# CODEJIN/multi_speaker_tts

Hardware: AMD Instinct MI355X
Metric: mel-frames/sec (train step) at batch 32x(128 tok,800 mel) (higher is better)
Workload: dtype f32

## Files before the change

multi_speaker_tts_amd/csrc/gemm_split.inc:

```

typedef __bf16 gs_bf16x8 __attribute__((ext_vector_type(8)));
typedef __bf16 gs_bf16x4 __attribute__((ext_vector_type(4)));
constexpr int GS_BM = 128, GS_LD = 40;
constexpr int GS_PLANE = 128 * GS_LD;

struct Split3 { gs_bf16x4 hi, mid, lo; };
__device__ __forceinline__ uint32_t gs_cvt_pk(float a, float b) {
    uint32_t r;
    asm("v_cvt_pk_bf16_f32 %0, %1, %2" : "=v"(r) : "v"(a), "v"(b));
    return r;
}
__device__ __forceinline__ float gs_sub(float a, uint32_t b_bits) {
    float r;
    asm("v_sub_f32 %0, %1, %2" : "=v"(r) : "v"(a), "v"(b_bits));
    return r;
}
__device__ __forceinline__ void gs_split2(float x0, float x1, uint32_t& hi, uint32_t& mid, uint32_t& lo) {
    hi = gs_cvt_pk(x0, x1);
    x0 = gs_sub(x0, hi << 16); x1 = gs_sub(x1, hi & 0xffff0000u);
    mid = gs_cvt_pk(x0, x1);
    x0 = gs_sub(x0, mid << 16); x1 = gs_sub(x1, mid & 0xffff0000u);
    lo = gs_cvt_pk(x0, x1);
}
__device__ __forceinline__ Split3 gs_split4(float a, float b, float c, float d) {
    uint2 h, m, l;
    gs_split2(a, b, h.x, m.x, l.x);
    gs_split2(c, d, h.y, m.y, l.y);
    Split3 s;
    s.hi = __builtin_bit_cast(gs_bf16x4, h); s.mid = __builtin_bit_cast(gs_bf16x4, m); s.lo = __builtin_bit_cast(gs_bf16x4, l);
    return s;
}
template <int PLANE>
struct SplitPlanes {
    static __device__ __forceinline__ void put(__bf16* __restrict__ p, float a, float b, float c, float d) {
        const Split3 s = gs_split4(a, b, c, d);
        *reinterpret_cast<gs_bf16x4*>(p) = s.hi;
        *reinterpret_cast<gs_bf16x4*>(p + PLANE) = s.mid;
        *reinterpret_cast<gs_bf16x4*>(p + 2 * PLANE) = s.lo;
    }
};

template <bool VEC, bool WIN> using GsLoaderKC = TileLoaderKC<8, 4, 32, GS_LD, SplitPlanes<GS_PLANE>, VEC, WIN>;
template <bool VEC, bool WIN> using GsLoaderMC = TileLoaderMC<8, GS_LD, SplitPlanes<GS_PLANE>, VEC, WIN>;

#ifdef GS_STAMP
#define GS_BAR(slot) do { if (stamp) { const unsigned long long t0_ = __builtin_readcyclecounter(); gemm_barrier(); acc_wait += __builtin_readcyclecounter() - t0_; } else gemm_barrier(); } while (0)
#else
#define GS_BAR(slot) gemm_barrier()
#endif

__device__ __forceinline__ int tiles_m_of(const GemmArgs& g) { return (g.M + GS_BM - 1) / GS_BM; }
constexpr int GS_NPROD = 6;
constexpr int GS_BUF = 6 * GS_PLANE;
constexpr size_t GS_LDS_BYTES = 2 * GS_BUF * sizeof(__bf16);

constexpr int GS_THREADS = 768;
template <class LoadFn, class StoreFn>
__device__ __forceinline__ void gs_produce(LoadFn load, StoreFn store, __bf16* lds0, int kbeg, int nt2) {
    float4 r[2][4];
    load(r[0], kbeg);
    load(r[1], kbeg + BK);
    store(r[0], lds0);
    load(r[0], kbeg + 2 * BK);
    gemm_barrier();
    for (int t = 0; t < nt2; t += 2) {
        store(r[1], lds0 + GS_BUF);
        load(r[1], kbeg + (t + 3) * BK);
        gemm_barrier();
        store(r[0], lds0);
        load(r[0], kbeg + (t + 4) * BK);
        gemm_barrier();
    }
}

template <bool TA, bool TB, bool VEC, bool WIN>
__global__ __launch_bounds__(GS_THREADS) void gemm_split_kernel(GemmArgs g) {
    extern __shared__ __attribute__((aligned(16))) __bf16 gs_lds[];

    const int tiles_n = (g.N + BN - 1) / BN;
    int tile = blockIdx.x, piece = -1;
    if (tile < g.body) {
        tile = gemm_xcd_tile(tile, g.body);
    } else {
        const int u = tile - g.body;
        tile = g.body + u / g.tail_s;
        piece = u % g.tail_s;
    }
    int tile_m = tile / tiles_n, tile_n = tile % tiles_n;
    if (g.band > 0) {
        const int per_band = g.band * tiles_m_of(g), b = tile / per_band, r = tile - b * per_band;
        const int w = min(g.band, tiles_n - b * g.band);
        tile_m = r / w; tile_n = b * g.band + r - tile_m * w;
    }
    const int batch = blockIdx.z / g.split_k, split = blockIdx.z % g.split_k;
    const int m0 = tile_m * GS_BM, n0 = tile_n * BN;
    const int kbeg = piece >= 0 ? piece * g.tail_kps : split * g.k_per_split;
    const int kend = min(g.K, kbeg + (piece >= 0 ? g.tail_kps : g.k_per_split));
    const int nt = kend > kbeg ? (kend - kbeg + BK - 1) / BK : 0, nt2 = (nt + 1) & ~1;
    const int wave = __builtin_amdgcn_readfirstlane((int)(threadIdx.x >> 6));
#ifdef GS_STAMP
    const bool stamp = blockIdx.x == 0 && blockIdx.z == 0 && wave == 0 && g.bias != nullptr;
    unsigned long long acc_wait = 0, t_begin = __builtin_readcyclecounter(), w_begin = wall_clock64();
#endif

    if (wave >= 4) {
        using LA = typename std::conditional<TA, GsLoaderMC<VEC, WIN>, GsLoaderKC<VEC, WIN>>::type;
        using LB = typename std::conditional<TB, GsLoaderKC<VEC, false>, GsLoaderMC<VEC, false>>::type;
        if (wave < 8) {
            const int tid = threadIdx.x - 256;
            LA la;
            la.prepare(tid, g.A + (long)batch * g.stride_a, g.lda, m0, kbeg, g.M, g.win_T, g.win_C, g.win_pad, g.win_dil);
            gs_produce([&](float4 (&r)[4], int k) { la.load(tid, r, k, kend, g.lda, g.win_T, g.win_C, g.win_pad, g.win_dil); },
                       [&](const float4 (&r)[4], __bf16* dst) { la.store(tid, r, dst); }, gs_lds, kbeg, nt2);
        } else {
            const int tid = threadIdx.x - 512;
            LB lb;
            lb.prepare(tid, g.B + (long)batch * g.stride_b, g.ldb, n0, kbeg, g.N, 0, 1, 0, 1);
            gs_produce([&](float4 (&r)[4], int k) { lb.load(tid, r, k, kend, g.ldb, 0, 1, 0, 1); },
                       [&](const float4 (&r)[4], __bf16* dst) { lb.store(tid, r, dst); }, gs_lds + 3 * GS_PLANE, kbeg, nt2);
        }
        return;
    }

    float* C = g.C + (long)batch * g.stride_c;
    const int lane = threadIdx.x & 63;
    const int wrow = (wave >> 1) * 64, wcol = (wave & 1) * 64;
    const int l31 = lane & 31, kg = lane >> 5;

    f32x16 acc[2][2];
#pragma unroll
    for (int i = 0; i < 2; ++i)
#pragma unroll
        for (int j = 0; j < 2; ++j)
#pragma unroll
            for (int r = 0; r < 16; ++r) acc[i][j][r] = 0.f;

    const int aoff = (wrow + l31) * GS_LD + kg * 8, boff = 3 * GS_PLANE + (wcol + l31) * GS_LD + kg * 8;
    gs_bf16x8 fa[2][2][3], fb[2][2][3];
    auto frags = [&](int set, const __bf16* buf, int ks) {
#pragma unroll
        for (int p = 0; p < 3; ++p) {
#pragma unroll
            for (int i = 0; i < 2; ++i) fa[set][i][p] = *reinterpret_cast<const gs_bf16x8*>(buf + aoff + p * GS_PLANE + i * 32 * GS_LD + ks * 16);
#pragma unroll
            for (int j = 0; j < 2; ++j) fb[set][j][p] = *reinterpret_cast<const gs_bf16x8*>(buf + boff + p * GS_PLANE + j * 32 * GS_LD + ks * 16);
        }
    };
    auto products = [&](int set) {
#pragma unroll
        for (int tt = 0; tt < GS_NPROD; ++tt) {
            const int pa = (tt == 0) ? 0 : (tt == 1) ? 1 : (tt == 2) ? 0 : (tt == 3) ? 1 : (tt == 4) ? 2 : 0;
            const int pb = (tt == 0) ? 0 : (tt == 1) ? 0 : (tt == 2) ? 1 : (tt == 3) ? 1 : (tt == 4) ? 0 : 2;
#pragma unroll
            for (int i = 0; i < 2; ++i)
#pragma unroll
                for (int j = 0; j < 2; ++j)
                    acc[i][j] = __builtin_amdgcn_mfma_f32_32x32x16_bf16(fa[set][i][pa], fb[set][j][pb], acc[i][j], 0, 0, 0);
        }
    };
    GS_BAR(0);
    frags(0, gs_lds, 0);
    for (int t = 0; t < nt2; ++t) {
        const __bf16* buf = gs_lds + (t & 1) * GS_BUF;
        frags(1, buf, 1);
        __builtin_amdgcn_sched_barrier(0);
        products(0);
        __builtin_amdgcn_sched_barrier(0);
        GS_BAR(0);
        frags(0, gs_lds + ((t + 1) & 1) * GS_BUF, 0);
        __builtin_amdgcn_sched_barrier(0);
        products(1);
        __builtin_amdgcn_sched_barrier(0);
    }
#ifdef GS_STAMP
    if (stamp && (threadIdx.x & 63) == 0) { unsigned long long* o = (unsigned long long*)g.bias; o[0] = acc_wait; o[1] = __builtin_readcyclecounter() - t_begin; o[2] = nt2; o[3] = wall_clock64() - w_begin; }
    if (stamp) return;
#endif
    gemm_store_tile<2, 2>(g, acc, C, m0 + wrow, n0 + wcol, lane, split == 0 && piece <= 0, g.split_k > 1 || piece >= 0);
}

constexpr int GSB_BM = 256, GSB_BN = 256, GSB_BK = 16, GSB_LD = 24, GSB_THREADS = 512;
constexpr int GSB_PLANE = 256 * GSB_LD;
constexpr int GSB_BUF = 6 * GSB_PLANE;
constexpr size_t GSB_LDS_BYTES = 2 * GSB_BUF * sizeof(__bf16);
template <bool VEC, bool WIN> using GsbLoaderKC = TileLoaderKC<4, 2, 128, GSB_LD, SplitPlanes<GSB_PLANE>, VEC, WIN>;
template <bool VEC, bool WIN> using GsbLoaderMC = TileLoaderMC<4, GSB_LD, SplitPlanes<GSB_PLANE>, VEC, WIN>;

template <bool TRANSPOSED, int HALF>
__device__ __forceinline__ bool gsb_stages(int tid) {
    if (TRANSPOSED) return (tid >> 8) == HALF;
    return true;
}

template <bool TA, bool TB, bool VEC, bool WIN>
__global__ __launch_bounds__(GSB_THREADS) void gemm_split_big_kernel(GemmArgs g) {
    extern __shared__ __attribute__((aligned(16))) __bf16 gs_lds[];
    const int tiles_n = (g.N + GSB_BN - 1) / GSB_BN;
    const int tile = gemm_xcd_tile(blockIdx.x, gridDim.x);
    const int tile_m = tile / tiles_n, tile_n = tile % tiles_n;
    const int batch = blockIdx.z / g.split_k, split = blockIdx.z % g.split_k;
    float* C = g.C + (long)batch * g.stride_c;
    const int m0 = tile_m * GSB_BM, n0 = tile_n * GSB_BN;
    const int kbeg = split * g.k_per_split;
    const int kend = min(g.K, kbeg + g.k_per_split);
    const int nt = kend > kbeg ? (kend - kbeg + GSB_BK - 1) / GSB_BK : 0;
    const int tid = threadIdx.x, lane = tid & 63, wave = __builtin_amdgcn_readfirstlane(tid >> 6);
    const int wrow = (wave >> 2) * 128, wcol = (wave & 3) * 64;
    const int l31 = lane & 31, kg = lane >> 5;

    using LA = typename std::conditional<TA, GsbLoaderMC<VEC, WIN>, GsbLoaderKC<VEC, WIN>>::type;
    using LB = typename std::conditional<TB, GsbLoaderKC<VEC, false>, GsbLoaderMC<VEC, false>>::type;
    LA la; LB lb;
    const bool a_mine = gsb_stages<TA, 0>(tid), b_mine = gsb_stages<!TB, 1>(tid);
    const int tid_a = TA ? (tid & 255) : tid, tid_b = TB ? tid : (tid & 255);
    if (a_mine) la.prepare(tid_a, g.A + (long)batch * g.stride_a, g.lda, m0, kbeg, g.M, g.win_T, g.win_C, g.win_pad, g.win_dil);
    if (b_mine) lb.prepare(tid_b, g.B + (long)batch * g.stride_b, g.ldb, n0, kbeg, g.N, 0, 1, 0, 1);
    float4 ra[4], rb[4];
    auto load = [&](int k) {
        if (a_mine) la.load(tid_a, ra, k, kend, g.lda, g.win_T, g.win_C, g.win_pad, g.win_dil);
        if (b_mine) lb.load(tid_b, rb, k, kend, g.ldb, 0, 1, 0, 1);
    };
    auto store = [&](int buf) {
        if (a_mine) la.store(tid_a, ra, gs_lds + buf * GSB_BUF);
        if (b_mine) lb.store(tid_b, rb, gs_lds + buf * GSB_BUF + 3 * GSB_PLANE);
    };

    f32x16 acc[4][2];
#pragma unroll
    for (int i = 0; i < 4; ++i)
#pragma unroll
        for (int j = 0; j < 2; ++j)
#pragma unroll
            for (int r = 0; r < 16; ++r) acc[i][j][r] = 0.f;

    const int aoff = (wrow + l31) * GSB_LD + kg * 8, boff = 3 * GSB_PLANE + (wcol + l31) * GSB_LD + kg * 8;
    gs_bf16x8 fb[2][3], fa0[4], fa1[4];
    auto ldA = [&](gs_bf16x8 (&f)[4], const __bf16* buf, int p) {
#pragma unroll
        for (int i = 0; i < 4; ++i) f[i] = *reinterpret_cast<const gs_bf16x8*>(buf + aoff + p * GSB_PLANE + i * 32 * GSB_LD);
    };
    auto ldB = [&](const __bf16* buf) {
#pragma unroll
        for (int p = 0; p < 3; ++p)
#pragma unroll
            for (int j = 0; j < 2; ++j) fb[j][p] = *reinterpret_cast<const gs_bf16x8*>(buf + boff + p * GSB_PLANE + j * 32 * GSB_LD);
    };
    auto mm = [&](const gs_bf16x8 (&f)[4], int pb) {
#pragma unroll
        for (int i = 0; i < 4; ++i)
#pragma unroll
            for (int j = 0; j < 2; ++j)
                acc[i][j] = __builtin_amdgcn_mfma_f32_32x32x16_bf16(f[i], fb[j][pb], acc[i][j], 0, 0, 0);
    };

    if (nt > 0) {
        load(kbeg);
        store(0);
        load(kbeg + GSB_BK);
        gemm_barrier();
        for (int t = 0; t < nt; ++t) {
            const __bf16* buf = gs_lds + (t & 1) * GSB_BUF;
            ldB(buf); ldA(fa0, buf, 0); ldA(fa1, buf, 1);
            mm(fa0, 0); mm(fa0, 1); mm(fa0, 2);
            ldA(fa0, buf, 2);
            store((t + 1) & 1);
            load(kbeg + (t + 2) * GSB_BK);
            mm(fa1, 0); mm(fa1, 1);
            mm(fa0, 0);
            gemm_barrier();
        }
    }
    gemm_store_tile<4, 2>(g, acc, C, m0 + wrow, n0 + wcol, lane, split == 0, g.split_k > 1);
}

struct GemmSplit {
    using Args = GemmArgs;
    static constexpr int THREADS = GS_THREADS;
    static constexpr size_t LDS_BYTES = GS_LDS_BYTES;
    template <bool TA, bool TB, bool VEC, bool WIN> static constexpr auto kernel() { return &gemm_split_kernel<TA, TB, VEC, WIN>; }
};
struct GemmSplitBig {
    using Args = GemmArgs;
    static constexpr int THREADS = GSB_THREADS;
    static constexpr size_t LDS_BYTES = GSB_LDS_BYTES;
    template <bool TA, bool TB, bool VEC, bool WIN> static constexpr auto kernel() { return &gemm_split_big_kernel<TA, TB, VEC, WIN>; }
};
```

multi_speaker_tts_amd/csrc/gemm_tile.h:

```cpp
#pragma once
#include "common.h"
#include <utility>

namespace mstts {

typedef float f32x16 __attribute__((ext_vector_type(16)));

struct GemmTileArgs {
    const float* A; const float* B; float* C; const float* bias;
    int M, N, K;
    long lda, ldb, ldc;
    int win_T, win_C, win_pad, win_dil;
    int act, accumulate, split_k;
    long stride_a, stride_b, stride_c;
    float alpha;
    int k_per_split;
};

__device__ __forceinline__ float apply_act(float v, int act) {
    if (act == MSTTS_ACT_RELU) return fmaxf(v, 0.f);
    if (act == MSTTS_ACT_TANH) return tanhf_(v);
    if (act == MSTTS_ACT_SIGMOID) return sigmoidf_(v);
    return v;
}

static __device__ __attribute__((aligned(16))) const float gemm_zero16[4] = {0.f, 0.f, 0.f, 0.f};
typedef float gemm_f32x4 __attribute__((ext_vector_type(4)));
typedef const gemm_f32x4 __attribute__((address_space(1)))* gemm_gptr4;
__device__ __forceinline__ float4 gemm_ld4(const float* p) {
    const gemm_f32x4 v = *(gemm_gptr4)p;
    return make_float4(v[0], v[1], v[2], v[3]);
}

__device__ __forceinline__ void gemm_barrier() { asm volatile("s_waitcnt lgkmcnt(0)\n\ts_barrier" ::: "memory"); }

constexpr int gemm_log2(int v) { return v <= 1 ? 0 : 1 + gemm_log2(v >> 1); }

template <int KQ, int NV, int RSTEP, int LD, class Stage, bool VEC, bool WIN>
struct TileLoaderKC {
    static constexpr int BKT = 4 * KQ, KSH = gemm_log2(KQ);
    const float* ubase;
    unsigned voff[NV], rmask;
    int t_row[NV], tap, kc, ld_;
    __device__ __forceinline__ void prepare(int tid, const float* __restrict__ base, long ld, int row0, int k0, int rows, int wT, int wC, int wpad, int wdil) {
        const int k4 = tid & (KQ - 1), r = tid >> KSH;
        rmask = 0; ld_ = (int)ld;
#pragma unroll
        for (int i = 0; i < NV; ++i) {
            const int row = row0 + r + i * RSTEP;
            if (row < rows) rmask |= 1u << i;
            voff[i] = (unsigned)((r + i * RSTEP) * (int)ld) + (WIN ? 0u : (unsigned)(k4 * 4));
            if (WIN) t_row[i] = row % wT;
        }
        if (WIN) {
            const int k = k0 + k4 * 4;
            tap = k / wC; kc = k - tap * wC;
            ubase = base + ((long)row0 - (long)wpad * wdil) * ld;
        } else {
            ubase = base + (long)row0 * ld + k0;
        }
    }
    __device__ __forceinline__ void load(int tid, float4 (&reg)[4], int k0, int kmax, long, int wT, int wC, int wpad, int wdil) {
        const int k4 = tid & (KQ - 1);
        const int k = k0 + k4 * 4;
        const bool kok = k < kmax;
        const int sh = WIN ? (tap - wpad) * wdil : 0;
        const unsigned wadd = WIN ? (unsigned)(tap * wdil * ld_ + kc) : 0u;
#pragma unroll
        for (int i = 0; i < NV; ++i) {
            float4 v = make_float4(0.f, 0.f, 0.f, 0.f);
            bool ok = kok && ((rmask >> i) & 1u);
            if (WIN) {
                const int t = t_row[i] + sh;
                ok = ok && t >= 0 && t < wT;
            }
            if (VEC) {
                v = gemm_ld4(ok ? ubase + (voff[i] + wadd) : gemm_zero16);
            } else if (ok) {
                const float* p = ubase + (voff[i] + wadd);
                v.x = p[0];
                if (k + 1 < kmax) v.y = p[1];
                if (k + 2 < kmax) v.z = p[2];
                if (k + 3 < kmax) v.w = p[3];
            }
            reg[i] = v;
        }
        if (WIN) {
            kc += BKT;
            const bool wrap = kc >= wC;
            kc -= wrap ? wC : 0; tap += wrap ? 1 : 0;
        } else {
            ubase += BKT;
        }
    }
    __device__ __forceinline__ void store(int tid, const float4 (&reg)[4], __bf16* __restrict__ s) const {
        const int k4 = tid & (KQ - 1), r = tid >> KSH;
#pragma unroll
        for (int i = 0; i < NV; ++i) Stage::put(s + (r + i * RSTEP) * LD + k4 * 4, reg[i].x, reg[i].y, reg[i].z, reg[i].w);
    }
};

template <int KQ, int LD, class Stage, bool VEC, bool WIN>
struct TileLoaderMC {
    static constexpr int BKT = 4 * KQ, KSH = gemm_log2(KQ);
    const float* ubase;
    unsigned voff[4];
    int sh, t_k[4], cols_left;
    __device__ __forceinline__ void prepare(int tid, const float* __restrict__ base, long ld, int col0, int k0, int cols, int wT, int wC, int wpad, int wdil) {
        const int kq = tid & (KQ - 1), c4 = tid >> KSH;
        const int col = col0 + c4 * 4;
        cols_left = cols - col;
        if (WIN) {
            const int tp = col / wC, cm = col - tp * wC;
            sh = (tp - wpad) * wdil;
#pragma unroll
            for (int i = 0; i < 4; ++i) {
                t_k[i] = (k0 + kq * 4 + i) % wT;
                voff[i] = (unsigned)((kq * 4 + i + tp * wdil) * (int)ld + cm);
            }
            ubase = base + ((long)k0 - (long)wpad * wdil) * ld;
        } else {
            sh = 0;
#pragma unroll
            for (int i = 0; i < 4; ++i) voff[i] = (unsigned)((kq * 4 + i) * (int)ld + c4 * 4);
            ubase = base + (long)k0 * ld + col0;
        }
    }
    __device__ __forceinline__ void load(int tid, float4 (&reg)[4], int k0, int kmax, long ld, int wT, int, int, int) {
        const int kq = tid & (KQ - 1);
#pragma unroll
        for (int i = 0; i < 4; ++i) {
            const int k = k0 + kq * 4 + i;
            float4 v = make_float4(0.f, 0.f, 0.f, 0.f);
            bool ok = k < kmax && cols_left > 0;
            if (WIN) {
                const int t = t_k[i] + sh;
                ok = ok && t >= 0 && t < wT;
                t_k[i] += BKT;
                t_k[i] -= (t_k[i] >= wT) ? wT : 0;
            }
            if (VEC) {
                v = gemm_ld4(ok ? ubase + voff[i] : gemm_zero16);
            } else if (ok) {
                const float* p = ubase + voff[i];
                v.x = p[0];
                if (cols_left > 1) v.y = p[1];
                if (cols_left > 2) v.z = p[2];
                if (cols_left > 3) v.w = p[3];
            }
            reg[i] = v;
        }
        ubase += BKT * ld;
    }
    __device__ __forceinline__ void store(int tid, const float4 (&reg)[4], __bf16* __restrict__ s) const {
        const int kq = tid & (KQ - 1), c4 = tid >> KSH;
        __bf16* p = s + (c4 * 4) * LD + kq * 4;
        Stage::put(p, reg[0].x, reg[1].x, reg[2].x, reg[3].x);
        Stage::put(p + LD, reg[0].y, reg[1].y, reg[2].y, reg[3].y);
        Stage::put(p + 2 * LD, reg[0].z, reg[1].z, reg[2].z, reg[3].z);
        Stage::put(p + 3 * LD, reg[0].w, reg[1].w, reg[2].w, reg[3].w);
    }
};

__device__ __forceinline__ int gemm_xcd_tile(int tile, int nb) {
    const int q = nb >> 3, r = nb & 7, xcd = tile & 7, idx = tile >> 3;
    if (nb >= 64) tile = xcd * q + (xcd < r ? xcd : r) + idx;
    return tile;
}

template <int WM, int WN>
__device__ __forceinline__ void gemm_store_tile(const GemmTileArgs& g, const f32x16 (&acc)[WM][WN], float* __restrict__ C, int row0, int col0,
                                                int lane, bool with_bias, bool atomic) {
#pragma unroll
    for (int i = 0; i < WM; ++i)
#pragma unroll
        for (int j = 0; j < WN; ++j) {
            const int col = col0 + j * 32 + (lane & 31);
            if (col >= g.N) continue;
            const float bv = (g.bias != nullptr && with_bias) ? g.bias[col] : 0.f;
#pragma unroll
            for (int r = 0; r < 16; ++r) {
                const int row = row0 + i * 32 + (r & 3) + 8 * (r >> 2) + 4 * (lane >> 5);
                if (row >= g.M) continue;
                float v = g.alpha * acc[i][j][r] + bv;
                float* dst = C + (long)row * g.ldc + col;
                if (atomic) {
                    atomicAdd(dst, v);
                } else {
                    v = apply_act(v, g.act);
                    if (g.accumulate) v += *dst;
                    *dst = v;
                }
            }
        }
}

static inline int gemm_k_per_split(int K, int split, int bk) {
    const int kps = ((K + split - 1) / split + bk - 1) / bk * bk;
    return kps < bk ? bk : kps;
}

static inline int gemm_args_from(const mstts_gemm_desc* d, const char* who, int bk, long max_ld, GemmTileArgs* g, bool* vec) {
    MSTTS_REQUIRE(d != nullptr, MSTTS_ERR_SHAPE, "%s: null descriptor", who);
    MSTTS_REQUIRE(d->M >= 0 && d->N >= 0 && d->K >= 0, MSTTS_ERR_SHAPE, "%s: negative dims", who);
    if (d->M == 0 || d->N == 0) { g->M = g->N = 0; return MSTTS_OK; }
    MSTTS_REQUIRE(d->A && d->B && d->C, MSTTS_ERR_SHAPE, "%s: null operand", who);
    MSTTS_REQUIRE(d->M < (1LL << 31) && d->N < (1LL << 31) && d->K < (1LL << 31), MSTTS_ERR_SHAPE, "%s: dims exceed int32", who);
    MSTTS_REQUIRE(max_ld <= 0 || (d->lda >= 0 && d->ldb >= 0 && d->lda < max_ld && d->ldb < max_ld), MSTTS_ERR_SHAPE,
                  "%s: row strides must be below 2^24 elements (tile-relative offsets are 32-bit)", who);
    const int split = d->split_k > 1 ? d->split_k : 1;
    MSTTS_REQUIRE(split == 1 || (d->act == MSTTS_ACT_NONE), MSTTS_ERR_SHAPE,
                  "%s: split_k needs act=none (output must be pre-zeroed or accumulated into)", who);
    if (d->win_T > 0) {
        MSTTS_REQUIRE(d->win_C > 0 && d->lda == d->win_C, MSTTS_ERR_SHAPE, "%s: window mode needs lda == win_C", who);
        MSTTS_REQUIRE(d->win_C % 4 == 0, MSTTS_ERR_SHAPE, "%s: window mode needs win_C %% 4 == 0", who);
    }
    g->A = d->A; g->B = d->B; g->C = d->C; g->bias = d->bias;
    g->M = (int)d->M; g->N = (int)d->N; g->K = (int)d->K;
    g->lda = d->lda; g->ldb = d->ldb; g->ldc = d->ldc;
    g->win_T = d->win_T; g->win_C = d->win_C > 0 ? d->win_C : 1; g->win_pad = d->win_pad; g->win_dil = d->win_dil > 0 ? d->win_dil : 1;
    g->act = d->act; g->accumulate = d->accumulate; g->split_k = split;
    g->stride_a = d->stride_a; g->stride_b = d->stride_b; g->stride_c = d->stride_c;
    g->alpha = d->alpha;
    g->k_per_split = gemm_k_per_split(g->K, split, bk);
    bool v = aligned16(d->A) && aligned16(d->B) && (d->lda % 4 == 0) && (d->ldb % 4 == 0) &&
             (d->stride_a % 4 == 0) && (d->stride_b % 4 == 0);
    v = v && (d->trans_a ? (d->M % 4 == 0) : (d->K % 4 == 0));
    v = v && (d->trans_b ? (d->K % 4 == 0) : (d->N % 4 == 0));
    if (d->win_T > 0) v = v && (d->win_C % 4 == 0);
    *vec = v;
    return MSTTS_OK;
}

template <class F> using GemmKernelFn = void (*)(typename F::Args);
template <class F, size_t... I>
static const GemmKernelFn<F>* gemm_kernel_table(std::index_sequence<I...>) {
    static const GemmKernelFn<F> table[16] = {F::template kernel<(I & 8) != 0, (I & 4) != 0, (I & 2) != 0, (I & 1) != 0>()...};
    return table;
}
template <class F>
static const GemmKernelFn<F>* gemm_kernel_table() { return gemm_kernel_table<F>(std::make_index_sequence<16>()); }
template <class F>
static int gemm_ready() {
    static int memo[64];
    int dev = 0;
    if (hipGetDevice(&dev) != hipSuccess || dev < 0 || dev >= 64) return 0;
    if (!memo[dev]) {
        bool ok = true;
        for (int i = 0; i < 16; ++i)
            ok = ok && hipFuncSetAttribute((const void*)gemm_kernel_table<F>()[i], hipFuncAttributeMaxDynamicSharedMemorySize, (int)F::LDS_BYTES) == hipSuccess;
        if (!ok) (void)hipGetLastError();
        memo[dev] = ok ? 2 : 1;
    }
    return memo[dev] == 2;
}
template <class F>
static void gemm_launch(const typename F::Args& g, bool ta, bool tb, bool vec, bool win, dim3 grid, hipStream_t st) {
    const int variant = (ta ? 8 : 0) + (tb ? 4 : 0) + (vec ? 2 : 0) + (win ? 1 : 0);
    hipLaunchKernelGGL(gemm_kernel_table<F>()[variant], grid, dim3(F::THREADS), F::LDS_BYTES, st, g);
}

}
```

Before: 639,900.

## Switch split-bf16 GEMM consumer to 16x16x32 MFMA with swizzled LDS layout

Adds a compile-time option (on by default for the 128-tile split GEMM) that swaps 32x32x16 bf16 MFMAs for 16x16x32 ones. It rewrites fragment loading and the product schedule, interleaving LDS reads of the hi/mid/lo planes between MFMA groups. An XOR swizzle on the K offset is added to the tile loaders to cut LDS bank conflicts, plus a new 16x16 store epilogue. The consumer barrier now waits only on LDS counters, and the big-tile kernel gets an optional path that stays off by default. The risks are higher register pressure from 16 accumulators per wave and a different MFMA throughput profile.

Measured after the change: 642,900, median of 6. Within noise of the previous version (+0.5%).

```diff
diff --git a/multi_speaker_tts_amd/csrc/gemm_split.inc b/multi_speaker_tts_amd/csrc/gemm_split.inc
--- a/multi_speaker_tts_amd/csrc/gemm_split.inc
+++ b/multi_speaker_tts_amd/csrc/gemm_split.inc
@@ -40,13 +40,30 @@
     }
 };
 
-template <bool VEC, bool WIN> using GsLoaderKC = TileLoaderKC<8, 4, 32, GS_LD, SplitPlanes<GS_PLANE>, VEC, WIN>;
-template <bool VEC, bool WIN> using GsLoaderMC = TileLoaderMC<8, GS_LD, SplitPlanes<GS_PLANE>, VEC, WIN>;
-
+#ifndef GS_MFMA_K
+#define GS_MFMA_K 32
+#endif
+static_assert(GS_MFMA_K == 16 || GS_MFMA_K == 32, "GS_MFMA_K: 16 (v_mfma_f32_32x32x16_bf16) or 32 (v_mfma_f32_16x16x32_bf16)");
+struct GsRows16 {
+    static __device__ __forceinline__ int k(int row, int k) { return k ^ ((row + 4) & 8); }
+};
+#if GS_MFMA_K == 32
+using GsRows = GsRows16;
+#else
+using GsRows = PlainRows;
+#endif
+template <bool VEC, bool WIN> using GsLoaderKC = TileLoaderKC<8, 4, 32, GS_LD, SplitPlanes<GS_PLANE>, VEC, WIN, GsRows>;
+template <bool VEC, bool WIN> using GsLoaderMC = TileLoaderMC<8, GS_LD, SplitPlanes<GS_PLANE>, VEC, WIN, GsRows>;
+
+#if GS_MFMA_K == 32
+__device__ __forceinline__ void gs_consumer_barrier() { __builtin_amdgcn_s_waitcnt(0xc07f); asm volatile("s_barrier" ::: "memory"); }
+#else
+__device__ __forceinline__ void gs_consumer_barrier() { gemm_barrier(); }
+#endif
 #ifdef GS_STAMP
-#define GS_BAR(slot) do { if (stamp) { const unsigned long long t0_ = __builtin_readcyclecounter(); gemm_barrier(); acc_wait += __builtin_readcyclecounter() - t0_; } else gemm_barrier(); } while (0)
-#else
-#define GS_BAR(slot) gemm_barrier()
+#define GS_BAR(slot) do { if (stamp) { const unsigned long long t0_ = __builtin_readcyclecounter(); gs_consumer_barrier(); acc_wait += __builtin_readcyclecounter() - t0_; } else gs_consumer_barrier(); } while (0)
+#else
+#define GS_BAR(slot) gs_consumer_barrier()
 #endif
 
 __device__ __forceinline__ int tiles_m_of(const GemmArgs& g) { return (g.M + GS_BM - 1) / GS_BM; }
@@ -125,6 +142,56 @@
     float* C = g.C + (long)batch * g.stride_c;
     const int lane = threadIdx.x & 63;
     const int wrow = (wave >> 1) * 64, wcol = (wave & 1) * 64;
+#if GS_MFMA_K == 32
+    const int l15 = lane & 15, kg = lane >> 4;
+    f32x4 acc[4][4];
+#pragma unroll
+    for (int i = 0; i < 4; ++i)
+#pragma unroll
+        for (int j = 0; j < 4; ++j)
+#pragma unroll
+            for (int r = 0; r < 4; ++r) acc[i][j][r] = 0.f;
+
+    const int koff = GsRows::k(l15, kg * 8);
+    const int aoff = (wrow + l15) * GS_LD + koff, boff = 3 * GS_PLANE + (wcol + l15) * GS_LD + koff;
+    gs_bf16x8 ah[4], am[4], al[4], bh[4], bm[4], bl[4];
+    auto rd = [&](gs_bf16x8 (&f)[4], const __bf16* buf, int off, int p) {
+#pragma unroll
+        for (int i = 0; i < 4; ++i) f[i] = *reinterpret_cast<const gs_bf16x8*>(buf + off + p * GS_PLANE + i * 16 * GS_LD);
+    };
+    auto mm = [&](const gs_bf16x8 (&a)[4], const gs_bf16x8 (&b)[4]) {
+#pragma unroll
+        for (int i = 0; i < 4; ++i)
+#pragma unroll
+            for (int j = 0; j < 4; ++j)
+                acc[i][j] = __builtin_amdgcn_mfma_f32_16x16x32_bf16(a[i], b[j], acc[i][j], 0, 0, 0);
+        __builtin_amdgcn_sched_barrier(0);
+    };
+    GS_BAR(0);
+    rd(al, gs_lds, aoff, 2); rd(bh, gs_lds, boff, 0); rd(ah, gs_lds, aoff, 0); rd(bl, gs_lds, boff, 2);
+    __builtin_amdgcn_sched_barrier(0);
+    for (int t = 0; t < nt2; ++t) {
+        const __bf16* buf = gs_lds + (t & 1) * GS_BUF;
+        const __bf16* nxt = gs_lds + ((t + 1) & 1) * GS_BUF;
+        mm(al, bh);
+        rd(am, buf, aoff, 1); rd(bm, buf, boff, 1);
+        __builtin_amdgcn_sched_barrier(0);
+        mm(ah, bh);
+        GS_BAR(0);
+        rd(al, nxt, aoff, 2);
+        __builtin_amdgcn_sched_barrier(0);
+        mm(am, bh);
+        rd(bh, nxt, boff, 0);
+        __builtin_amdgcn_sched_barrier(0);
+        mm(ah, bl);
+        rd(bl, nxt, boff, 2);
+        __builtin_amdgcn_sched_barrier(0);
+        mm(ah, bm);
+        rd(ah, nxt, aoff, 0);
+        __builtin_amdgcn_sched_barrier(0);
+        mm(am, bm);
+    }
+#else
     const int l31 = lane & 31, kg = lane >> 5;
 
     f32x16 acc[2][2];
@@ -172,19 +239,33 @@
         products(1);
         __builtin_amdgcn_sched_barrier(0);
     }
+#endif
 #ifdef GS_STAMP
     if (stamp && (threadIdx.x & 63) == 0) { unsigned long long* o = (unsigned long long*)g.bias; o[0] = acc_wait; o[1] = __builtin_readcyclecounter() - t_begin; o[2] = nt2; o[3] = wall_clock64() - w_begin; }
     if (stamp) return;
 #endif
+#if GS_MFMA_K == 32
+    gemm_store_tile16<4, 4>(g, acc, C, m0 + wrow, n0 + wcol, lane, split == 0 && piece <= 0, g.split_k > 1 || piece >= 0);
+#else
     gemm_store_tile<2, 2>(g, acc, C, m0 + wrow, n0 + wcol, lane, split == 0 && piece <= 0, g.split_k > 1 || piece >= 0);
+#endif
 }
 
 constexpr int GSB_BM = 256, GSB_BN = 256, GSB_BK = 16, GSB_LD = 24, GSB_THREADS = 512;
 constexpr int GSB_PLANE = 256 * GSB_LD;
 constexpr int GSB_BUF = 6 * GSB_PLANE;
 constexpr size_t GSB_LDS_BYTES = 2 * GSB_BUF * sizeof(__bf16);
-template <bool VEC, bool WIN> using GsbLoaderKC = TileLoaderKC<4, 2, 128, GSB_LD, SplitPlanes<GSB_PLANE>, VEC, WIN>;
-template <bool VEC, bool WIN> using GsbLoaderMC = TileLoaderMC<4, GSB_LD, SplitPlanes<GSB_PLANE>, VEC, WIN>;
+#ifndef GSB_MFMA_K
+#define GSB_MFMA_K 16
+#endif
+static_assert(GSB_MFMA_K == 16 || GSB_MFMA_K == 32, "GSB_MFMA_K: 16 (v_mfma_f32_32x32x16_bf16) or 32 (v_mfma_f32_16x16x32_bf16)");
+#if GSB_MFMA_K == 32
+using GsbRows = GsRows16;
+#else
+using GsbRows = PlainRows;
+#endif
+template <bool VEC, bool WIN> using GsbLoaderKC = TileLoaderKC<4, 2, 128, GSB_LD, SplitPlanes<GSB_PLANE>, VEC, WIN, GsbRows>;
+template <bool VEC, bool WIN> using GsbLoaderMC = TileLoaderMC<4, GSB_LD, SplitPlanes<GSB_PLANE>, VEC, WIN, GsbRows>;
 
 template <bool TRANSPOSED, int HALF>
 __device__ __forceinline__ bool gsb_stages(int tid) {
@@ -206,7 +287,9 @@
     const int nt = kend > kbeg ? (kend - kbeg + GSB_BK - 1) / GSB_BK : 0;
     const int tid = threadIdx.x, lane = tid & 63, wave = __builtin_amdgcn_readfirstlane(tid >> 6);
     const int wrow = (wave >> 2) * 128, wcol = (wave & 3) * 64;
+#if GSB_MFMA_K == 16
     const int l31 = lane & 31, kg = lane >> 5;
+#endif
 
     using LA = typename std::conditional<TA, GsbLoaderMC<VEC, WIN>, GsbLoaderKC<VEC, WIN>>::type;
     using LB = typename std::conditional<TB, GsbLoaderKC<VEC, false>, GsbLoaderMC<VEC, false>>::type;
@@ -225,6 +308,56 @@
         if (b_mine) lb.store(tid_b, rb, gs_lds + buf * GSB_BUF + 3 * GSB_PLANE);
     };
 
+#if GSB_MFMA_K == 32
+    const int l15 = lane & 15, up = lane >> 5;
+    f32x4 acc[8][4];
+#pragma unroll
+    for (int i = 0; i < 8; ++i)
+#pragma unroll
+        for (int j = 0; j < 4; ++j)
+#pragma unroll
+            for (int r = 0; r < 4; ++r) acc[i][j][r] = 0.f;
+
+    const int koff = GsbRows::k(l15, ((lane >> 4) & 1) * 8);
+    const int aoff = (wrow + l15) * GSB_LD + koff, boff = 3 * GSB_PLANE + (wcol + l15) * GSB_LD + koff;
+    const int a1 = aoff + up * GSB_PLANE, a2 = aoff + up * 2 * GSB_PLANE, b3 = boff + (1 - up) * 2 * GSB_PLANE;
+    gs_bf16x8 fa[8], fb[4];
+    auto ldA = [&](const __bf16* buf, int off) {
+#pragma unroll
+        for (int i = 0; i < 8; ++i) fa[i] = *reinterpret_cast<const gs_bf16x8*>(buf + off + i * 16 * GSB_LD);
+    };
+    auto ldB = [&](gs_bf16x8 (&f)[4], const __bf16* buf, int off) {
+#pragma unroll
+        for (int j = 0; j < 4; ++j) f[j] = *reinterpret_cast<const gs_bf16x8*>(buf + off + j * 16 * GSB_LD);
+    };
+    auto mm = [&](const gs_bf16x8 (&f)[4]) {
+#pragma unroll
+        for (int i = 0; i < 8; ++i)
+#pragma unroll
+            for (int j = 0; j < 4; ++j)
+                acc[i][j] = __builtin_amdgcn_mfma_f32_16x16x32_bf16(fa[i], f[j], acc[i][j], 0, 0, 0);
+    };
+
+    if (nt > 0) {
+        load(kbeg);
+        store(0);
+        load(kbeg + GSB_BK);
+        gemm_barrier();
+        for (int t = 0; t < nt; ++t) {
+            const __bf16* buf = gs_lds + (t & 1) * GSB_BUF;
+            ldB(fb, buf, boff); ldA(buf, a1);
+            mm(fb);
+            ldB(fb, buf, boff + GSB_PLANE);
+            store((t + 1) & 1);
+            load(kbeg + (t + 2) * GSB_BK);
+            mm(fb);
+            ldB(fb, buf, b3); ldA(buf, a2);
+            mm(fb);
+            gemm_barrier();
+        }
+    }
+    gemm_store_tile16<8, 4>(g, acc, C, m0 + wrow, n0 + wcol, lane, split == 0, g.split_k > 1);
+#else
     f32x16 acc[4][2];
 #pragma unroll
     for (int i = 0; i < 4; ++i)
@@ -271,6 +404,7 @@
         }
     }
     gemm_store_tile<4, 2>(g, acc, C, m0 + wrow, n0 + wcol, lane, split == 0, g.split_k > 1);
+#endif
 }
 
 struct GemmSplit {
diff --git a/multi_speaker_tts_amd/csrc/gemm_tile.h b/multi_speaker_tts_amd/csrc/gemm_tile.h
--- a/multi_speaker_tts_amd/csrc/gemm_tile.h
+++ b/multi_speaker_tts_amd/csrc/gemm_tile.h
@@ -35,8 +35,11 @@
 __device__ __forceinline__ void gemm_barrier() { asm volatile("s_waitcnt lgkmcnt(0)\n\ts_barrier" ::: "memory"); }
 
 constexpr int gemm_log2(int v) { return v <= 1 ? 0 : 1 + gemm_log2(v >> 1); }
-
-template <int KQ, int NV, int RSTEP, int LD, class Stage, bool VEC, bool WIN>
+struct PlainRows {
+    static __device__ __forceinline__ int k(int, int k) { return k; }
+};
+
+template <int KQ, int NV, int RSTEP, int LD, class Stage, bool VEC, bool WIN, class Rows = PlainRows>
 struct TileLoaderKC {
     static constexpr int BKT = 4 * KQ, KSH = gemm_log2(KQ);
     const float* ubase;
@@ -96,11 +99,11 @@
     __device__ __forceinline__ void store(int tid, const float4 (&reg)[4], __bf16* __restrict__ s) const {
         const int k4 = tid & (KQ - 1), r = tid >> KSH;
 #pragma unroll
-        for (int i = 0; i < NV; ++i) Stage::put(s + (r + i * RSTEP) * LD + k4 * 4, reg[i].x, reg[i].y, reg[i].z, reg[i].w);
-    }
-};
-
-template <int KQ, int LD, class Stage, bool VEC, bool WIN>
+        for (int i = 0; i < NV; ++i) Stage::put(s + (r + i * RSTEP) * LD + Rows::k(r + i * RSTEP, k4 * 4), reg[i].x, reg[i].y, reg[i].z, reg[i].w);
+    }
+};
+
+template <int KQ, int LD, class Stage, bool VEC, bool WIN, class Rows = PlainRows>
 struct TileLoaderMC {
     static constexpr int BKT = 4 * KQ, KSH = gemm_log2(KQ);
     const float* ubase;
@@ -154,7 +157,7 @@
     }
     __device__ __forceinline__ void store(int tid, const float4 (&reg)[4], __bf16* __restrict__ s) const {
         const int kq = tid & (KQ - 1), c4 = tid >> KSH;
-        __bf16* p = s + (c4 * 4) * LD + kq * 4;
+        __bf16* p = s + (c4 * 4) * LD + Rows::k(c4 * 4, kq * 4);
         Stage::put(p, reg[0].x, reg[1].x, reg[2].x, reg[3].x);
         Stage::put(p + LD, reg[0].y, reg[1].y, reg[2].y, reg[3].y);
         Stage::put(p + 2 * LD, reg[0].z, reg[1].z, reg[2].z, reg[3].z);
@@ -193,6 +196,34 @@
                 }
             }
         }
+}
+
+typedef float f32x4 __attribute__((ext_vector_type(4)));
+template <int WM, int WN>
+__device__ __forceinline__ void gemm_store_tile16(const GemmTileArgs& g, const f32x4 (&acc)[WM][WN], float* __restrict__ C, int row0, int col0,
+                                                  int lane, bool with_bias, bool atomic) {
+#pragma unroll
+    for (int j = 0; j < WN; ++j) {
+        const int col = col0 + j * 16 + (lane & 15);
+        if (col >= g.N) continue;
+        const float bv = (g.bias != nullptr && with_bias) ? g.bias[col] : 0.f;
+#pragma unroll
+        for (int i = 0; i < WM; ++i)
+#pragma unroll
+            for (int r = 0; r < 4; ++r) {
+                const int row = row0 + i * 16 + 4 * (lane >> 4) + r;
+                if (row >= g.M) continue;
+                float v = g.alpha * acc[i][j][r] + bv;
+                float* dst = C + (long)row * g.ldc + col;
+                if (atomic) {
+                    atomicAdd(dst, v);
+                } else {
+                    v = apply_act(v, g.act);
+                    if (g.accumulate) v += *dst;
+                    *dst = v;
+                }
+            }
+    }
 }
 
 static inline int gemm_k_per_split(int K, int split, int bk) {
```
